# henry123-boy/Level-S2FM_official

Measured on AMD Instinct MI355X. Metric: rendered rays/sec (fwd+bwd), higher is better.
Workload: dtype f32; 1 GPU; C2: ETH3D bounds, 1024 rays x 128 samples per GPU, dual field, L16/F2/T19 hash grid, fwd+loss+bwd; rays_per_gpu=1024, samples_per_ray=128, dual_field=True, parallelism=dp1 (rays sharded by view)

## Files before the change

### include/ls2fm.h

```cpp
#ifndef LS2FM_H
#define LS2FM_H

#include <stdint.h>

#ifdef __cplusplus
extern "C" {
#endif

#define LS2FM_ABI_VERSION 13
#define LS2FM_MAX_LEVELS 16
#define LS2FM_HIDDEN 64
#define LS2FM_FEAT 16
#define LS2FM_VIEW_ENC 27

typedef enum ls2fm_status {
    LS2FM_OK = 0,
    LS2FM_ERR_INVALID_ARGUMENT = -1,
    LS2FM_ERR_UNSUPPORTED = -2,
    LS2FM_ERR_LAUNCH = -3,
    LS2FM_ERR_WORKSPACE = -4,
    LS2FM_ERR_STARVED = -5
} ls2fm_status;

typedef struct ls2fm_grid_desc {
// ... 547 lines not shown
                        const int64_t* row, int64_t n_rows, float* points, float* normals, float* colours, int64_t* pixel,
                        void* stream);

#define LS2FM_TEXTURE_TILE 16
#define LS2FM_TEXTURE_MAX_CLASSES 8
int ls2fm_texture_texels(const float* verts, int64_t n_verts, const int32_t* faces, int64_t n_faces, const int32_t* order,
                         const int32_t* rot, int32_t n_classes, const int32_t* class_log2_pitch, const int64_t* class_count,
                         int32_t gutter, int32_t size, int32_t row_begin, int32_t row_end, int32_t* face, float* point,
                         float* normal, float* uv, void* stream);
int ls2fm_texture_render(const int32_t* face_id, const float* bary, int32_t n_views, int32_t height, int32_t width, const float* uv,
                         int64_t n_faces, const float* texture, int32_t size, int32_t channels, const float* background, float* out,
                         void* stream);

int ls2fm_set_scatter_mode(int mode);
int ls2fm_get_scatter_mode(void);

int ls2fm_profile_enable(int on);
int ls2fm_profile_reset(void);
int ls2fm_profile_count(void);
const char* ls2fm_profile_name(int index);
int ls2fm_profile_get(int index, double* total_ms, int64_t* launches);

#ifdef __cplusplus
}
#endif
#endif
```

### level-s2fm_official_amd/csrc/bin_items.h

```cpp
#pragma once

#include "render_common.h"

namespace {

constexpr int kAccSlots = 2 << kSlabShift;
constexpr int kSlabBins = 128 << (13 - kSlabShift);
constexpr int kBins = kSlabBins;
#ifndef LS2FM_FILL_TILE
#define LS2FM_FILL_TILE 256
#endif
constexpr int kCountThreads = LS2FM_FILL_TILE;
constexpr int kFillThreads = LS2FM_FILL_TILE;
constexpr int kFillCap = kFillThreads * 17 / 4;
#ifndef LS2FM_FILL_WIN
#define LS2FM_FILL_WIN (LS2FM_FILL_TILE * 17 / 8)
#endif
constexpr int kFillWin = LS2FM_FILL_WIN;
#ifndef LS2FM_ACC_THREADS
#define LS2FM_ACC_THREADS 1024
#endif
constexpr int kAccThreads = LS2FM_ACC_THREADS;
#ifndef LS2FM_ACC_BATCH
#define LS2FM_ACC_BATCH 4
#endif
constexpr int kAccBatch = LS2FM_ACC_BATCH;
constexpr int kMaxParts = 16;

typedef unsigned long long u64;

struct __attribute__((aligned(16))) Item {
    uint32_t ij;
    float wx;
    float a0, a1, b0, b1;
    float c0, c1;
};

struct __attribute__((aligned(4))) ItemS {
    uint32_t ij;
    float v00, v01;
    float v10, v11;
};
// ... 278 lines not shown
```

### level-s2fm_official_amd/csrc/bin_scatter.hip

```cpp
#include <atomic>
#include <cstdlib>

#include "bin_items.h"
#include "side_jobs.h"

namespace {

#ifndef LS2FM_FILL_MINW
#define LS2FM_FILL_MINW 5
#endif
template <bool DUAL>
__global__ void __launch_bounds__(kFillThreads, LS2FM_FILL_MINW)
scatter_fill_kernel(LevelSet lv, FieldC fc, const float* __restrict__ center, const float* __restrict__ ray, int64_t n_points,
                    int64_t p_pad, int sshift, const float* __restrict__ rpt, const float* __restrict__ rec1,
                    const float* __restrict__ rec2, const float* __restrict__ ray_bound, int64_t n_rays, int64_t r_pad,
                    BinMeta bm, int level_base, int n_explicit, SideJobs sj) {
    typedef typename ItemOf<DUAL>::type ItemT;
    __shared__ int hist[kBins];
    __shared__ int lds_off[kBins];
    __shared__ int base[kBins];
    __shared__ int run_len[kBins];
    constexpr int kWin = DUAL ? kFillWin : kFillCap;
    constexpr int kItemBytes = kWin * (int)sizeof(ItemT);
    constexpr int kStageBytes = kItemBytes + 4 * kWin + (DUAL ? 4 * kWin : 0);
    constexpr int kRawBytes = kStageBytes > 4 * kTailArenaFloats ? kStageBytes : 4 * kTailArenaFloats;
    static_assert(kItemBytes % 16 == 0, "the index array behind the items is aligned");
    __shared__ __attribute__((aligned(16))) unsigned char s_raw[kRawBytes];
    ItemT* const s_items = reinterpret_cast<ItemT*>(s_raw);
    uint32_t* const s_gidx = reinterpret_cast<uint32_t*>(s_raw + kItemBytes);
// ... 9 lines not shown
    const int tid = threadIdx.x, lane = tid & 63, l = level_base + n_lv - 1 - y_lv;
    const int n_tiles_x = (int)gridDim.x;
    const int tile_x = (n_tiles_x & 7) == 0 ? ((int)blockIdx.x & 7) * (n_tiles_x >> 3) + ((int)blockIdx.x >> 3) : (int)blockIdx.x;
    if (tile_x == 0 && y_lv == 0) {
        if (tid == 0) *acc_claim(bm) = 0;
        for (int q = tid; q < LS2FM_MAX_LEVELS * kBins; q += kFillThreads) bm.part_ticket[q] = 0;
    }
    static_assert(kBins <= kFillThreads, "one thread per slab for the run offsets");
    int pre_base = 0;
    if (tid < kBins) {
        const int before = bm.tile[((int64_t)l * bm.n_tiles + tile_x) * kBins + tid];
        pre_base = bm.start[l * kBins + tid] + before;
    }
    for (int b = tid; b < kBins; b += kFillThreads) hist[b] = 0;
    __syncthreads();
    const LevelC L = make_level_c(lv, l, sshift);
    const int64_t i = (int64_t)tile_x * kFillThreads + tid;
    const bool live = i < n_points;
    uint32_t g[3] = {0u, 0u, 0u};
    float w[3] = {0.f, 0.f, 0.f}, d0 = 0.f, d1 = 0.f, r0 = 0.f, r1 = 0.f, e0 = 0.f, e1 = 0.f, qd[3] = {0.f, 0.f, 0.f};
    if (live) {
        const float4 a = reinterpret_cast<const float4*>(rpt)[2 * i];
        const float4 c = reinterpret_cast<const float4*>(rpt)[2 * i + 1];
        const float4 b = reinterpret_cast<const float4*>(rec1)[(int64_t)l * p_pad + i];
        const float x[3] = {a.x, a.y, a.z};
#pragma unroll
        for (int q = 0; q < 3; ++q) pos_fract(x[q], L.scale, g[q], w[q]);
        d0 = b.x; d1 = b.y; r0 = b.z; r1 = b.w;
        qd[0] = L.scale * a.w; qd[1] = L.scale * c.x; qd[2] = L.scale * c.y;
        if (DUAL) {
            const float2 e = reinterpret_cast<const float2*>(rec2)[(int64_t)l * p_pad + i];
// ... 194 lines not shown
            for (int o = 32; o > 0; o >>= 1) b = fmaxf(b, __shfl_xor(b, o, 64));
            if (lane == 0) red[tid >> 6] = b;
            __syncthreads();
            if (tid == 0) {
                float m = 0.f;
                for (int q = 0; q < kFillThreads / 64; ++q) m = fmaxf(m, red[q]);
                bm.level_bound[16 * which + l] = m;
            }
            __syncthreads();
        }
    }
}

struct SlabPlan {
    int first[LS2FM_MAX_LEVELS + 1];
    int parts[LS2FM_MAX_LEVELS];
    int scratch[LS2FM_MAX_LEVELS];
    int headroom_bits;
    int n_explicit;
};

constexpr int kMinHeadroomBits = 18;
__device__ __forceinline__ void add_fixed(u64* slot, float v, float to_fixed) {
    const double d = fma((double)v, (double)to_fixed, 6755399441055744.0);
    atomicAdd(slot, (u64)__double_as_longlong(d) - 0x4338000000000000ull);
}

__device__ __forceinline__ void quantum_of(float bound, int headroom_bits, float& to_fixed, double& to_float) {
    int e_bound = 0;
    if (bound > 0.f) (void)frexpf(bound, &e_bound);
    int shift = 62 - headroom_bits - e_bound;
    shift = shift > 126 ? 126 : (shift < -126 ? -126 : shift);
    to_fixed = ldexpf(1.0f, shift);
    to_float = ldexp(1.0, -shift);
}

#ifdef LS2FM_STAMPS
__device__ long long g_acc_stamps[8 * 4096];
#endif


template <bool DUAL, bool ADD_INTO>
__device__ __forceinline__ void combine_entry(const LevelSet& lv, const SlabPlan& plan, const BinMeta& bm, int sshift, float* __restrict__ dtable1,
                                              float* __restrict__ dtable2, int l, uint32_t slab, int entry, float bound1, float bound2) {
    constexpr int F = DUAL ? 4 : 2;
    const uint32_t lo = slab << sshift;
    const uint32_t hi = lo + (1u << sshift) < lv.size[l] ? lo + (1u << sshift) : lv.size[l];
    if (lo + (uint32_t)entry >= hi) return;
    const int parts = plan.parts[l];
    float to_fixed, to_fixed2;
    double to_float1, to_float2;
    quantum_of(bound1, plan.headroom_bits, to_fixed, to_float1);
    quantum_of(bound2, plan.headroom_bits, to_fixed2, to_float2);
    const int E = 1 << sshift;
    const u64* __restrict__ src = bm.part_acc + (size_t)(plan.scratch[l] + (int)slab * parts) * kAccSlots + entry;
    u64 tot[F];
#pragma unroll
    for (int f = 0; f < F; ++f) tot[f] = 0ull;
    constexpr int kCombineBatch = 4;
    for (int q0 = 0; q0 < parts; q0 += kCombineBatch) {
        u64 v[kCombineBatch][F];
#pragma unroll
// ... 220 lines not shown
            }
#pragma unroll
            for (int u = 0; u < kAccBatch; ++u)
                if (b0 + tid + u * kAccThreads < cur.j_hi) add_item(now[u], DUAL ? nowx[u] : 0.f);
            b0 += BT;
        } while (b0 < cur.j_hi);
        PACC_STAMP(cur.uid, 1);
        if (tid < 64) {
            asm volatile("s_waitcnt vmcnt(0)" : "+v"(claimed) :: "memory");
            if (tid == 0) s_claim = claimed;
        }
        lds_barrier();
        PACC_STAMP(cur.uid, 2);
        AccUnitRaw nraw = acc_unit_fetch<DUAL, true>(plan, bm, block_base, dyn_base + __builtin_amdgcn_readfirstlane(s_claim), dyn_end);
        const uint32_t size = lv.size[l];
        const uint32_t lo = cur.slab << sshift;
        const uint32_t hi = lo + (1u << sshift) < size ? lo + (1u << sshift) : size;
        if (cur.parts > 1 && combine) {
            if (!(ADD_INTO && cur.n_items == 0)) {
                uint4* mine = reinterpret_cast<uint4*>(bm.part_acc + (size_t)(plan.scratch[l] + cur.wg) * kAccSlots);
                const uint4 z = make_uint4(0u, 0u, 0u, 0u);
                for (int e = tid; e < kAccSlots / 2; e += kAccThreads) {
                    mine[e] = reinterpret_cast<const uint4*>(acc)[e];
                    reinterpret_cast<uint4*>(acc)[e] = z;
                }
                __syncthreads();
                if (tid == 0) {
                    __builtin_amdgcn_fence(__ATOMIC_RELEASE, "agent");
                    asm volatile("s_waitcnt vmcnt(0)" ::: "memory");
                    const int arrived = __hip_atomic_fetch_add(&bm.part_ticket[l * kBins + (int)cur.slab], 1, __ATOMIC_RELAXED, __HIP_MEMORY_SCOPE_AGENT);
                    const int last = arrived == cur.parts - 1;
                    if (last) __builtin_amdgcn_fence(__ATOMIC_ACQUIRE, "agent");
                    s_claim2 = last;
                }
                __syncthreads();
                if (s_claim2) {
                    for (int entry = tid; entry < E; entry += kAccThreads)
                        combine_entry<DUAL, ADD_INTO>(lv, plan, bm, sshift, dtable1, dtable2, l, cur.slab, entry, cur.bound1, cur.bound2);
                }
            }
        } else if (!(ADD_INTO && cur.n_items == 0)) {
            float* dst1 = dtable1 + 2ull * (lv.offset[l] + lo);
            float* dst2 = DUAL ? dtable2 + 2ull * (lv.offset[l] + lo) : nullptr;
            for (int entry = tid; entry < (int)(hi - lo); entry += kAccThreads) {
                u64 tot[F];
#pragma unroll
                for (int f = 0; f < F; ++f) { tot[f] = acc[f * E + entry]; acc[f * E + entry] = 0ull; }
                float2 v1 = make_float2((float)((double)(long long)tot[0] * to_float1), (float)((double)(long long)tot[1] * to_float1));
                float* d1 = dst1 + 2 * entry;
                if (cur.parts > 1) {
                    if (tot[0] != 0ull) atomicAdd(d1, v1.x);
                    if (tot[1] != 0ull) atomicAdd(d1 + 1, v1.y);
// ... 55 lines not shown
        while (n < grid->n_levels && n < kMaxExplicitLevels && (long long)grid->resolution[n] <= n_samples) ++n;
    if (n > kMaxExplicitLevels) n = kMaxExplicitLevels;
    if (n > grid->n_levels) n = grid->n_levels;
    return n;
}

size_t ls2fm_bin_counts_bytes() { return 0; }

bool ls2fm_bins_levels_fit(const ls2fm_grid_desc* grid, int dual) { return levels_fit(grid, ls2fm_slab_shift(dual)); }

int ls2fm_launch_scatter_fill(const ls2fm_grid_desc* grid, const FieldC& fc, const float* center, const float* ray, float* bins_ws,
                              int64_t n_points, int64_t p_pad, const float* rec1, const float* rec2, const float* rpt,
                              const float* ray_bound, int64_t n_rays, int dual, hipStream_t stream, int level_lo, int level_hi,
                              int n_explicit, const void* side_jobs) {
    const int64_t r_pad = (n_rays + 63) / 64 * 64;
    const int sshift = ls2fm_slab_shift(dual);
    const BinMeta bm = make_bin_meta(bins_ws, n_points);
    const LevelSet lv = make_level_set(grid);
    if (level_hi < 0) level_hi = grid->n_levels;
    if (level_hi <= level_lo) return LS2FM_OK;
    SideJobs sj{};
    if (side_jobs) {
        sj = *static_cast<const SideJobs*>(side_jobs);
        const int n_jobs = sj.dec_blocks + sj.l1_jobs + sj.n_red + kFinalizeTasks;
        sj.rows = (n_jobs + bm.n_tiles - 1) / bm.n_tiles;
    }
    if (kFillThreads != kWmThreads && sj.rows > 0) return LS2FM_ERR_UNSUPPORTED;
    const dim3 g((unsigned)bm.n_tiles, (unsigned)(level_hi - level_lo + sj.rows));
    if (dual) scatter_fill_kernel<true><<<g, kFillThreads, 0, stream>>>(lv, fc, center, ray, n_points, p_pad, sshift, rpt, rec1, rec2, ray_bound, n_rays, r_pad, bm, level_lo, n_explicit, sj);
    else      scatter_fill_kernel<false><<<g, kFillThreads, 0, stream>>>(lv, fc, center, ray, n_points, p_pad, sshift, rpt, rec1, nullptr, ray_bound, n_rays, r_pad, bm, level_lo, 0, sj);
    return ls2fm_launch_status();
}

namespace {
struct HostPlan { SlabPlan plan; int total, zero_lo, zero_hi; };

std::atomic<int> g_scatter_mode{[] { const char* e = getenv("LS2FM_SCATTER_MODE"); return e ? atoi(e) : 1; }()};

HostPlan make_plan(const ls2fm_grid_desc* grid, int64_t n_points, int sshift, int n_explicit = 0, int n_samples = 1) {
    const int capacity = part_blocks_capacity(n_points);
    for (int max_parts = kMaxParts;; --max_parts) {
        HostPlan h{};
        for (int l = 0; l < LS2FM_MAX_LEVELS; ++l) h.plan.parts[l] = 1;
        h.plan.headroom_bits = 4;
        while ((1ll << (h.plan.headroom_bits - 4)) < n_points) ++h.plan.headroom_bits;
        if (h.plan.headroom_bits < kMinHeadroomBits) h.plan.headroom_bits = kMinHeadroomBits;
        h.plan.n_explicit = n_explicit < LS2FM_MAX_LEVELS ? n_explicit : 0;
        h.zero_lo = h.zero_hi = -1;
        const int64_t target = 16384;
        int scratch = 0;
        for (int l = 0; l < LS2FM_MAX_LEVELS + 1; ++l) {
            h.plan.first[l] = h.total;
            if (l >= grid->n_levels) continue;
            const int slabs = level_slabs(grid->size[l], sshift);
            int parts = 1;
            if (!grid->hashed[l] || slabs < 16) {
                int64_t per_block = 4 * n_points / slabs;
                if (l < n_explicit) {
                    const double run = 0.9 * (double)n_samples / (double)grid->resolution[l];
                    if (run > 1.0) per_block = (int64_t)((double)per_block / run);
                }
                parts = (int)((per_block + target - 1) / target);
                if (parts > max_parts) parts = max_parts;
                if (parts < 1) parts = 1;
            }
            h.plan.parts[l] = parts;
            h.plan.scratch[l] = scratch;
            if (parts > 1) {
                scratch += slabs * parts;
                if (h.zero_lo < 0) h.zero_lo = l;
                h.zero_hi = l;
            }
            h.total += slabs * parts;
        }
        if (scratch <= capacity || max_parts == 1) return h;
    }
}
}

extern "C" int ls2fm_set_scatter_mode(int mode) {
    if (mode != 0 && mode != 1) return LS2FM_ERR_INVALID_ARGUMENT;
    g_scatter_mode.store(mode);
    return LS2FM_OK;
}
extern "C" int ls2fm_get_scatter_mode(void) { return g_scatter_mode.load(); }

void ls2fm_scatter_zero_range(const ls2fm_grid_desc* grid, int64_t n_points, bool dual, int64_t* first, int64_t* count) {
    const HostPlan h = make_plan(grid, n_points, ls2fm_slab_shift(dual ? 1 : 0));
    *first = 0; *count = 0;
    if (g_scatter_mode.load() != 0 || h.zero_lo < 0) return;
    *first = grid->offset[h.zero_lo];
    *count = (int64_t)grid->offset[h.zero_hi] + grid->size[h.zero_hi] - *first;
}

#ifdef LS2FM_STAMPS
extern "C" int ls2fm_debug_acc_stamps(long long* host) {
    return hipMemcpyFromSymbol(host, HIP_SYMBOL(g_acc_stamps), sizeof(long long) * 8 * 4096) == hipSuccess ? 0 : -1;
}
#endif

int ls2fm_launch_slab_accumulate(const ls2fm_grid_desc* grid, float* bins_ws, int64_t n_points, float* dtable1, float* dtable2,
                                 hipStream_t stream, int level_lo, int level_hi, int add_into, int n_explicit, int n_samples) {
    const bool dual = dtable2 != nullptr;
    const int sshift = ls2fm_slab_shift(dual ? 1 : 0);
    const BinMeta bm = make_bin_meta(bins_ws, n_points);
    const LevelSet lv = make_level_set(grid);
    const HostPlan h = make_plan(grid, n_points, sshift, dual ? n_explicit : LS2FM_MAX_LEVELS, n_samples);
    const int combine = g_scatter_mode.load() != 0 ? 1 : 0;
    if (level_hi < 0) level_hi = grid->n_levels;
    const int base = h.plan.first[level_lo], blocks = h.plan.first[level_hi] - base;
    if (blocks <= 0) return LS2FM_OK;
    static const int n_cus = [] {
        int dev = 0, n = 0;
        if (hipGetDevice(&dev) != hipSuccess || hipDeviceGetAttribute(&n, hipDeviceAttributeMultiprocessorCount, dev) != hipSuccess || n < 1) n = 256;
        return n;
    }();
    {
        const int g = blocks < n_cus ? blocks : n_cus;
        int* claim = acc_claim(bm);
        int hold = 0;
        for (int l = level_lo; l < level_hi && h.plan.parts[l] > 1; ++l) hold += h.plan.first[l + 1] - h.plan.first[l];
        if (hold > g || blocks < 3 * g) hold = 0;
// ... 12 lines not shown
```

### level-s2fm_official_amd/csrc/render_common.h

```cpp
#pragma once

#include "ls2fm_device.h"

enum ls2fm_prof_id {
    LS2FM_PROF_PREP = 0, LS2FM_PROF_ENCODE_SDF, LS2FM_PROF_ENCODE_RAD, LS2FM_PROF_SHADE_FWD, LS2FM_PROF_SHADE_BWD,
    LS2FM_PROF_WGRAD_GEO, LS2FM_PROF_WGRAD_TAIL, LS2FM_PROF_SCATTER_SDF, LS2FM_PROF_SCATTER_RAD, LS2FM_PROF_FINALIZE,
    LS2FM_PROF_SDF_EVAL, LS2FM_PROF_SPHERE_TRACE, LS2FM_PROF_BIN, LS2FM_PROF_LOSS_FWD,
    LS2FM_PROF_LOSS_BWD, LS2FM_PROF_WGRAD_MLP, LS2FM_PROF_POSE, LS2FM_PROF_ENCODE_PAIR,
    LS2FM_PROF_BALM_LINEARIZE, LS2FM_PROF_BALM_POINTS, LS2FM_PROF_BALM_SCHUR, LS2FM_PROF_BALM_SOLVE, LS2FM_PROF_BALM_BACKSUB,
    LS2FM_PROF_BALM_COST, LS2FM_PROF_COUNT
};
bool ls2fm_prof_enabled();
void ls2fm_prof_begin(int id, hipStream_t stream);
void ls2fm_prof_end(int id, hipStream_t stream);

struct SideCtx { hipStream_t side; hipEvent_t fork, mid, join; };
bool ls2fm_side_stream(SideCtx* out, hipStream_t caller);
int ls2fm_join_on_error(bool forked, const SideCtx& sc, hipStream_t caller, int status);
int* ls2fm_async_error_word(hipStream_t stream);
int ls2fm_device_cus();

constexpr int kHidden = LS2FM_HIDDEN;
constexpr int kOut = LS2FM_FEAT + 1;
constexpr int kInMax = 3 + 2 * LS2FM_MAX_LEVELS;
// ... 166 lines not shown
int ls2fm_explicit_levels(const ls2fm_grid_desc* grid, int dual, int n_samples);

struct WsLayout {
    int64_t p, p_pad, r_pad;
    int l1, l2, dual;
    int64_t packed, e1, j1, e2, sdfv, nrm, rgbs, fe, fe2, rout, lpart;
    int64_t rec1, rec2, rpt, bins, v, p3, gf, dz, gf2, dzr, renc, dexyz, dlen, mpart, wg, dbeta, smax;
    int64_t total;
};

#ifndef LS2FM_SLAB_SHIFT
#define LS2FM_SLAB_SHIFT 13
#endif
constexpr int kSlabShift = LS2FM_SLAB_SHIFT;
static inline int ls2fm_slab_shift(int dual) { return dual ? kSlabShift - 1 : kSlabShift; }
constexpr int kWgradMlpBlocks = 256;
constexpr int kRegsSdf = 48 + 16 + 16 + 5;
constexpr int kRegsGeo = 48 + 16 + 4;
constexpr int kRegsDec = 20;
constexpr int kL1Seg = 16;
struct WgPartLayout {
    int64_t l1_sdf;
    int64_t l1_geo;
    int64_t dec;
    int64_t slot_sdf;
    int64_t slot_geo;
    int64_t total;
    int n_slots;
};
static inline bool ls2fm_fused_wgrad(int n_samples) {
// ... 137 lines not shown
```

### level-s2fm_official_amd/csrc/render_fwd.hip

```cpp
#include <cmath>

#include "bin_items.h"

namespace {

struct LayerRef { const float* v; const float* g; const float* b; int out, in; };

__device__ __forceinline__ LayerRef layer_ref(const ls2fm_params& P, int li, int in_dim, int rad_in) {
    switch (li) {
        case 0: return {P.sdf_mlp[0].weight_v, P.sdf_mlp[0].weight_g, P.sdf_mlp[0].bias, kHidden, in_dim};
        case 1: return {P.sdf_mlp[1].weight_v, P.sdf_mlp[1].weight_g, P.sdf_mlp[1].bias, kOut, kHidden};
        case 2: return {P.geo_mlp[0].weight_v, P.geo_mlp[0].weight_g, P.geo_mlp[0].bias, kHidden, in_dim};
        case 3: return {P.geo_mlp[1].weight_v, P.geo_mlp[1].weight_g, P.geo_mlp[1].bias, kOut, kHidden};
        case 4: return {P.rad_mlp[0].weight_v, P.rad_mlp[0].weight_g, P.rad_mlp[0].bias, kHidden, rad_in};
        case 5: return {P.rad_mlp[1].weight_v, P.rad_mlp[1].weight_g, P.rad_mlp[1].bias, kHidden, kHidden};
        default: return {P.rad_mlp[2].weight_v, P.rad_mlp[2].weight_g, P.rad_mlp[2].bias, 3, kHidden};
    }
}

__device__ __forceinline__ int row_base(int li) {
    switch (li) {
        case 0: return 0;
        case 1: return 64;
        case 2: return 81;
// ... 195 lines not shown
    prep_weights_task(P, in_dim, in_dim2, rad_in, dual, with_rad, out, (int)blockIdx.x, (int)threadIdx.x, kPrepThreads);
}

struct XcdPlan { int start[9]; };

#ifdef LS2FM_STAMPS
__device__ unsigned long long g_enc_ticks[2 * LS2FM_MAX_LEVELS + 24];
#endif

struct EncodeExtras {
    ls2fm_params params;
    int in_dim, in_dim2, rad_in, dual;
    Packed* packed;
    int* tile_counts;
    int* scan_ticket;
    int n_tiles, sshift;
    int n_explicit;
    int n_prep_tasks;
    const float* pts;
};

constexpr int kEncThreads = 512;
constexpr int kEncRows = kEncThreads / kFillTile;
static_assert(kEncThreads % kFillTile == 0, "a gather workgroup covers whole tiles");
constexpr int kEncReserved = 8;

struct LevelOne { float scale; uint32_t res, size, offset, hashed; };

__device__ __forceinline__ void locate_sample(const FieldC& fc, const float* __restrict__ center, const float* __restrict__ ray,
                                              const float* __restrict__ pts, int64_t i, const LevelOne& lv, uint32_t g[3], Cell& c) {
    float p[3], x[3];
// ... 13 lines not shown
    for (int d = 0; d < 3; ++d) pos_fract(x[d], lv.scale, g[d], c.w[d]);
#pragma unroll
    for (int k = 0; k < 8; ++k)
        c.idx[k] = lv.offset + corner_index(g[0] + (k & 1), g[1] + ((k >> 1) & 1), g[2] + ((k >> 2) & 1), lv.res, lv.size,
                                            lv.hashed);
}

#ifndef LS2FM_ENC_MINW
#define LS2FM_ENC_MINW 1
#endif
template <bool INTERLEAVED>
__global__ void __launch_bounds__(kEncThreads, LS2FM_ENC_MINW)
ray_encode_kernel(LevelSet lv1, LevelSet lv2, FieldC fc, const float* __restrict__ center, const float* __restrict__ ray,
                  const float* __restrict__ table1, const float* __restrict__ table2, int64_t n_points, int64_t p_pad,
                  int n_chunks, XcdPlan plan, float* __restrict__ enc1, float* __restrict__ enc2, float* __restrict__ jac,
                  EncodeExtras ex) {
    __shared__ int hist[kEncRows][kBins];
    const int tid = threadIdx.x;
    if (blockIdx.x < kEncReserved) {
        if (ex.packed && (int)blockIdx.x < ex.n_prep_tasks)
            prep_weights_task(ex.params, ex.in_dim, ex.in_dim2, ex.rad_in, ex.dual, 1, ex.packed, (int)blockIdx.x, tid, kEncThreads);
        if (blockIdx.x == 3 && tid == 0 && ex.scan_ticket) *ex.scan_ticket = 0;
        return;
    }
    const int bx = (int)blockIdx.x - kEncReserved;
    const int xcd = bx & 7, j = bx >> 3;
    const int unit = plan.start[xcd] + j;
    if (unit >= plan.start[xcd + 1]) return;
    const int pl = unit / n_chunks;
    const int chunk = unit % n_chunks;
    const bool two = !INTERLEAVED && table2 != nullptr;
    const bool second = two && (pl & 1);
    const int l = two ? pl >> 1 : pl;
    LevelOne lv;
    lv.scale = second ? lv2.scale[l] : lv1.scale[l];
    lv.res = second ? lv2.res[l] : lv1.res[l];
    lv.size = second ? lv2.size[l] : lv1.size[l];
    lv.offset = second ? lv2.offset[l] : lv1.offset[l];
    lv.hashed = second ? lv2.hashed[l] : lv1.hashed[l];
    const bool counting = ex.tile_counts != nullptr && !second;
    if (counting) {
        for (int b = tid; b < kEncRows * kBins; b += kEncThreads) (&hist[0][0])[b] = 0;
        __syncthreads();
    }
    const int64_t i = (int64_t)chunk * kEncThreads + tid;
#ifdef LS2FM_STAMPS
    const long long t_begin = wall_clock64();
#endif
    if (i < n_points) {
        uint32_t g[3];
        Cell c;
        locate_sample(fc, center, ray, ex.pts, i, lv, g, c);
        auto enc_at = [=](float* __restrict__ base, int row, uint32_t k) -> float* { return base + ((int64_t)row * p_pad + i) * k; };
        if (INTERLEAVED) {
// ... 55 lines not shown
                    __builtin_nontemporal_store(lv.scale * g0, enc_at(jac, 2 * l + 0, 3u) + gd);
                    __builtin_nontemporal_store(lv.scale * g1, enc_at(jac, 2 * l + 1, 3u) + gd);
                }
            }
        }
        if (counting) {
            const bool factored = ex.dual != 0 && l >= ex.n_explicit;
            const int ray_len = ls2fm_ray_len_of_runs(ex.pts == nullptr, fc.n_samples);
            const uint32_t n_in_ray = ray_len != 0 ? (uint32_t)i % (uint32_t)ray_len : 0u;
            const RunFlags rf = wave_runs(g, true, tid & 63, factored ? kMergeMinDual : kMergeMinSingle, ray_len, n_in_ray);
            if (rf.head) {
                const bool halves = factored && rf.merged;
#pragma unroll
                for (int cp = 0; cp < 4; ++cp) {
                    const uint32_t i0 = c.idx[2 * cp] - lv.offset, i1 = c.idx[2 * cp + 1] - lv.offset;
                    const uint32_t s0 = i0 >> ex.sshift, s1 = i1 >> ex.sshift;
                    atomicAdd(&hist[tid / kFillTile][s0], 1);
                    if (s1 != s0 || halves) atomicAdd(&hist[tid / kFillTile][s1], 1);
                }
            }
        }
    }
    if (counting) {
        __syncthreads();
        for (int b = tid; b < kEncRows * kBins; b += kEncThreads) {
            const int tile = kEncRows * chunk + b / kBins;
            if (tile < ex.n_tiles) ex.tile_counts[((int64_t)l * ex.n_tiles + tile) * kBins + b % kBins] = hist[b / kBins][b % kBins];
        }
    }
#ifdef LS2FM_STAMPS
    __syncthreads();
// ... 118 lines not shown
int ls2fm_launch_points_encode(const ls2fm_field_desc* field, const ls2fm_grid_desc* grid, const ls2fm_params* params,
                               const float* pts, const WsLayout& w, float* ws, hipStream_t s) {
    const FieldC fc = make_field_c(field);
    const int L = grid->n_levels;
    const int n_chunks = (int)((w.p + kEncThreads - 1) / kEncThreads);
    int most = 0;
    const XcdPlan plan = make_xcd_plan(grid, L, nullptr, 0, 1, n_chunks, true, &most);
    EncodeExtras ex;
    ex.params = *params;
    ex.in_dim = 3 + 2 * L; ex.in_dim2 = 0; ex.rad_in = 0; ex.dual = 0;
    ex.packed = (Packed*)(ws + w.packed);
    const BinMeta bm = make_bin_meta(ws + w.bins, w.p);
    ex.tile_counts = bm.tile;
    ex.scan_ticket = scan_ticket(bm);
    ex.n_tiles = bm.n_tiles;
    ex.sshift = ls2fm_slab_shift(0);
    ex.n_explicit = 0;
    ex.n_prep_tasks = 1;
    ex.pts = pts;
    ray_encode_kernel<false><<<(unsigned)(kEncReserved + 8 * most), kEncThreads, 0, s>>>(
        make_level_set(grid), make_level_set(grid), fc, nullptr, nullptr, params->sdf_table, nullptr, w.p, w.p_pad, n_chunks, plan,
        ws + w.e1, nullptr, ws + w.j1, ex);
    return ls2fm_launch_status();
}
int ls2fm_launch_image_encode(const ls2fm_field_desc* field, const ls2fm_grid_desc* sdf_grid, const ls2fm_grid_desc* rad_grid,
                              const ls2fm_params* params, const float* center, const float* ray, int64_t n_points, int64_t p_pad,
                              float* e1, float* e2, float* j1, Packed* packed, hipStream_t s) {
    const FieldC fc = make_field_c(field);
    const int dual = field->dual_field ? 1 : 0;
    const int L1 = sdf_grid->n_levels, L2 = dual ? rad_grid->n_levels : 0;
    const int n_chunks = (int)((n_points + kEncThreads - 1) / kEncThreads);
    const bool interleaved = dual && params->dual_table;
    const bool pair = dual && !interleaved;
    int most = 0;
    const XcdPlan plan = make_xcd_plan(sdf_grid, L1, pair ? rad_grid : nullptr, pair ? L2 : 0, field->n_samples, n_chunks, false, &most,
                                       interleaved);
    EncodeExtras ex;
    ex.params = *params;
    ex.in_dim = 3 + 2 * L1; ex.in_dim2 = 3 + 2 * L2; ex.rad_in = 3 + 3 + kView + LS2FM_FEAT * (dual ? 2 : 1); ex.dual = dual;
    ex.packed = packed;
    ex.tile_counts = nullptr; ex.scan_ticket = nullptr; ex.n_tiles = 0; ex.sshift = ls2fm_slab_shift(dual);
    ex.n_explicit = 0;
    ex.n_prep_tasks = 3; ex.pts = nullptr;
    const unsigned enc_blocks = (unsigned)(kEncReserved + 8 * most);
    const int enc_span = dual ? LS2FM_PROF_ENCODE_PAIR : LS2FM_PROF_ENCODE_SDF;
    ls2fm_prof_begin(enc_span, s);
    if (interleaved)
        ray_encode_kernel<true><<<enc_blocks, kEncThreads, 0, s>>>(
            make_level_set(sdf_grid), make_level_set(sdf_grid), fc, center, ray, params->dual_table, nullptr, n_points, p_pad, n_chunks,
            plan, e1, e2, j1, ex);
    else
        ray_encode_kernel<false><<<enc_blocks, kEncThreads, 0, s>>>(
            make_level_set(sdf_grid), make_level_set(pair ? rad_grid : sdf_grid), fc, center, ray, params->sdf_table,
            pair ? params->rad_table : nullptr, n_points, p_pad, n_chunks, plan, e1, pair ? e2 : nullptr, j1, ex);
    ls2fm_prof_end(enc_span, s);
    return ls2fm_launch_status();
}

int ls2fm_launch_post_shade(const ls2fm_loss_spec* loss, const float* ray_part, int64_t n_rays, int n_samples,
                            const ls2fm_grid_desc* scan_grid, int64_t n_points, float* bins_ws, hipStream_t stream);

extern "C" int ls2fm_render_fwd(const ls2fm_field_desc* field, const ls2fm_grid_desc* sdf_grid,
                                const ls2fm_grid_desc* rad_grid, const ls2fm_params* params, const float* center,
                                const float* ray, int64_t n_rays, float* rgb, float* sdfs_volume, float* normals,
                                float* depth_mlp, float* normal_mlp, void* workspace, const ls2fm_render_opts* opts,
                                void* stream) {
    LS2FM_CHECK_ARG(render_config_ok(field, sdf_grid, rad_grid) && params && n_rays >= 0);
    if (field->bg_sdf) return LS2FM_ERR_UNSUPPORTED;
    if (field->dual_field && !same_grid_geometry(sdf_grid, rad_grid)) return LS2FM_ERR_UNSUPPORTED;
// ... 12 lines not shown
    float* ws = (float*)workspace;
    Packed* pk = (Packed*)(ws + w.packed);
    const FieldC fc = make_field_c(field);

    const int n_chunks = (int)((w.p + kEncThreads - 1) / kEncThreads);
    const bool interleaved = dual && params->dual_table;
    const bool pair = dual && !interleaved;
    const int enc_span = dual ? LS2FM_PROF_ENCODE_PAIR : LS2FM_PROF_ENCODE_SDF;
    int most = 0;
    const XcdPlan plan = make_xcd_plan(sdf_grid, L1, pair ? rad_grid : nullptr, pair ? L2 : 0, field->n_samples, n_chunks, prepare_bwd, &most,
                                       interleaved);
    EncodeExtras ex;
    ex.params = *params;
    ex.in_dim = 3 + 2 * L1; ex.in_dim2 = 3 + 2 * L2; ex.rad_in = 3 + 3 + kView + LS2FM_FEAT * (dual ? 2 : 1); ex.dual = dual;
    ex.packed = pk;
    ex.tile_counts = nullptr; ex.scan_ticket = nullptr; ex.n_tiles = 0; ex.sshift = ls2fm_slab_shift(dual);
    ex.n_explicit = ls2fm_explicit_levels(sdf_grid, dual, field->n_samples);
    ex.n_prep_tasks = 3; ex.pts = nullptr;
    if (prepare_bwd) {
        const BinMeta bm = make_bin_meta(ws + w.bins, w.p);
        ex.tile_counts = bm.tile;
        ex.scan_ticket = scan_ticket(bm);
        ex.n_tiles = bm.n_tiles;
    }
    const unsigned enc_blocks = (unsigned)(kEncReserved + 8 * most);
    ls2fm_prof_begin(enc_span, s);
    if (interleaved)
        ray_encode_kernel<true><<<enc_blocks, kEncThreads, 0, s>>>(
            make_level_set(sdf_grid), make_level_set(sdf_grid), fc, center, ray, params->dual_table, nullptr, w.p, w.p_pad, n_chunks,
            plan, ws + w.e1, ws + w.e2, ws + w.j1, ex);
    else
        ray_encode_kernel<false><<<enc_blocks, kEncThreads, 0, s>>>(
            make_level_set(sdf_grid), make_level_set(pair ? rad_grid : sdf_grid), fc, center, ray, params->sdf_table,
            pair ? params->rad_table : nullptr, w.p, w.p_pad, n_chunks, plan, ws + w.e1, pair ? ws + w.e2 : nullptr, ws + w.j1, ex);
    ls2fm_prof_end(enc_span, s);

    ls2fm_prof_begin(LS2FM_PROF_SHADE_FWD, s);
    ls2fm_launch_shade_fwd(fc, dual, 2 * L1, 2 * L2, pk, center, ray, n_rays, w, ws, rgb, sdfs_volume, normals, depth_mlp,
                           normal_mlp, loss, s);
    ls2fm_prof_end(LS2FM_PROF_SHADE_FWD, s);
    if (loss && opts->loss_inputs_ready && hipStreamWaitEvent(s, (hipEvent_t)opts->loss_inputs_ready, 0) != hipSuccess)
        return LS2FM_ERR_LAUNCH;
    ls2fm_prof_begin(LS2FM_PROF_BIN, s);
    const int st = ls2fm_launch_post_shade(loss, ws + w.lpart, n_rays, field->n_samples, prepare_bwd ? sdf_grid : nullptr, w.p,
                                           ws + w.bins, s);
    ls2fm_prof_end(LS2FM_PROF_BIN, s);
    if (st != LS2FM_OK) return st;
    return ls2fm_launch_status();
}
// ... 1 lines not shown
```

### level-s2fm_official_amd/ls2fm/_lib.py

```python
from __future__ import annotations

import ctypes
import os
from ctypes import POINTER, Structure, c_char_p, c_double, c_float, c_int32, c_int64, c_uint32, c_void_p

import torch

MAX_LEVELS = 16
HIDDEN = 64
FEAT = 16
ABI_VERSION = 13
MAX_RENDER_POINTS = 1 << 23

_HERE = os.path.dirname(os.path.abspath(__file__))
LIB_PATH = os.environ.get("LS2FM_LIB") or os.path.join(_HERE, "libls2fm_hip.so")


class GridDesc(Structure):
    _fields_ = [
        ("n_levels", c_int32),
        ("n_features", c_int32),
        ("scale", c_float * MAX_LEVELS),
        ("resolution", c_uint32 * MAX_LEVELS),
        ("size", c_uint32 * MAX_LEVELS),
# ... 239 lines not shown
                                   _P]),
    "ls2fm_mvs_plane_score": (c_int32, [_P, c_int32, c_int32, c_int32, _P, c_int32, _P, c_int32, _P, _P, c_int32, c_int32, c_float, c_float,
                                        c_int32, _P, _P, _P, _P]),
    "ls2fm_mvs_patchmatch_step": (c_int32, [_P, c_int32, c_int32, c_int32, _P, c_int32, _P, c_int32, _P, _P, c_int32, c_int32, c_float,
                                            c_float, c_int32, c_int32, c_int32, ctypes.c_uint32, c_float, c_float, c_float, _P, _P, _P, _P,
                                            _P, _P]),
    "ls2fm_mvs_fuse_mark": (c_int32, [_P, _P, c_int32, c_int32, c_int32, _P, c_int32, _P, _P, _P, c_float, c_float, c_float, c_float,
                                      c_int32, c_int32, _P, _P]),
    "ls2fm_mvs_fuse_emit": (c_int32, [_P, _P, _P, c_int32, c_int32, c_int32, c_int32, _P, c_int32, _P, _P, _P, _P, c_float, c_float,
                                      c_float, c_float, c_int32, c_int32, _P, _P, c_int64, _P, _P, _P, _P, _P]),
    "ls2fm_texture_texels": (c_int32, [_P, c_int64, _P, c_int64, _P, _P, c_int32, POINTER(c_int32), POINTER(c_int64), c_int32, c_int32,
                                       c_int32, c_int32, _P, _P, _P, _P, _P]),
    "ls2fm_texture_render": (c_int32, [_P, _P, c_int32, c_int32, c_int32, _P, c_int64, _P, c_int32, c_int32, POINTER(c_float), _P, _P]),
    "ls2fm_set_scatter_mode": (c_int32, [c_int32]),
    "ls2fm_get_scatter_mode": (c_int32, []),
    "ls2fm_profile_enable": (c_int32, [c_int32]),
    "ls2fm_profile_reset": (c_int32, []),
    "ls2fm_profile_count": (c_int32, []),
    "ls2fm_profile_name": (c_char_p, [c_int32]),
    "ls2fm_profile_get": (c_int32, [c_int32, POINTER(ctypes.c_double), POINTER(c_int64)]),
}
EXPORTED_SYMBOLS = tuple(_SIGNATURES)

_lib = None


def load() -> ctypes.CDLL:
    global _lib
    if _lib is not None:
        return _lib
# ... 82 lines not shown
```

Before: 2.559 million rays/s.

## Pick per-level slab shift to split heavily loaded dense levels into finer slabs

Replaces the single global slab shift with a per-level shift chosen by the host planner. For dense or small levels whose estimated items per slab exceed the unit target, the shift is lowered (down to a minimum, while the slab count fits in the bin array), which spreads hot dense-grid gradient accumulation across more slabs and fewer partial combines. The shifts are threaded through the fill, encode histogram and accumulate/combine kernels, and a diagnostic export of the plan is added. This costs extra host planning per launch and slightly larger kernel arguments, and if any kernel's slab indexing is not kept consistent it can bin items wrongly.

After: 2.576 million rays/s (median of 6 runs). About the same (+0.7%).

```diff
diff --git a/include/ls2fm.h b/include/ls2fm.h
--- a/include/ls2fm.h
+++ b/include/ls2fm.h
@@ -585,6 +585,7 @@
 
 int ls2fm_set_scatter_mode(int mode);
 int ls2fm_get_scatter_mode(void);
+int ls2fm_scatter_plan(const ls2fm_grid_desc* grid, int64_t n_points, int dual, int n_explicit, int n_samples, int32_t* out);
 
 int ls2fm_profile_enable(int on);
 int ls2fm_profile_reset(void);
diff --git a/level-s2fm_official_amd/csrc/bin_items.h b/level-s2fm_official_amd/csrc/bin_items.h
--- a/level-s2fm_official_amd/csrc/bin_items.h
+++ b/level-s2fm_official_amd/csrc/bin_items.h
@@ -26,6 +26,7 @@
 #endif
 constexpr int kAccBatch = LS2FM_ACC_BATCH;
 constexpr int kMaxParts = 16;
+constexpr int kMinSlabShift = 6;
 
 typedef unsigned long long u64;
 
diff --git a/level-s2fm_official_amd/csrc/bin_scatter.hip b/level-s2fm_official_amd/csrc/bin_scatter.hip
--- a/level-s2fm_official_amd/csrc/bin_scatter.hip
+++ b/level-s2fm_official_amd/csrc/bin_scatter.hip
@@ -12,7 +12,7 @@
 template <bool DUAL>
 __global__ void __launch_bounds__(kFillThreads, LS2FM_FILL_MINW)
 scatter_fill_kernel(LevelSet lv, FieldC fc, const float* __restrict__ center, const float* __restrict__ ray, int64_t n_points,
-                    int64_t p_pad, int sshift, const float* __restrict__ rpt, const float* __restrict__ rec1,
+                    int64_t p_pad, SlabShifts shifts, const float* __restrict__ rpt, const float* __restrict__ rec1,
                     const float* __restrict__ rec2, const float* __restrict__ ray_bound, int64_t n_rays, int64_t r_pad,
                     BinMeta bm, int level_base, int n_explicit, SideJobs sj) {
     typedef typename ItemOf<DUAL>::type ItemT;
@@ -52,7 +52,7 @@
     }
     for (int b = tid; b < kBins; b += kFillThreads) hist[b] = 0;
     __syncthreads();
-    const LevelC L = make_level_c(lv, l, sshift);
+    const LevelC L = make_level_c(lv, l, shifts.s[l]);
     const int64_t i = (int64_t)tile_x * kFillThreads + tid;
     const bool live = i < n_points;
     uint32_t g[3] = {0u, 0u, 0u};
@@ -277,6 +277,7 @@
 
 struct SlabPlan {
     int first[LS2FM_MAX_LEVELS + 1];
+    SlabShifts shift;
     int parts[LS2FM_MAX_LEVELS];
     int scratch[LS2FM_MAX_LEVELS];
     int headroom_bits;
@@ -307,8 +308,9 @@
 __device__ __forceinline__ void combine_entry(const LevelSet& lv, const SlabPlan& plan, const BinMeta& bm, int sshift, float* __restrict__ dtable1,
                                               float* __restrict__ dtable2, int l, uint32_t slab, int entry, float bound1, float bound2) {
     constexpr int F = DUAL ? 4 : 2;
-    const uint32_t lo = slab << sshift;
-    const uint32_t hi = lo + (1u << sshift) < lv.size[l] ? lo + (1u << sshift) : lv.size[l];
+    const int lshift = plan.shift.s[l];
+    const uint32_t lo = slab << lshift;
+    const uint32_t hi = lo + (1u << lshift) < lv.size[l] ? lo + (1u << lshift) : lv.size[l];
     if (lo + (uint32_t)entry >= hi) return;
     const int parts = plan.parts[l];
     float to_fixed, to_fixed2;
@@ -559,8 +561,9 @@
         PACC_STAMP(cur.uid, 2);
         AccUnitRaw nraw = acc_unit_fetch<DUAL, true>(plan, bm, block_base, dyn_base + __builtin_amdgcn_readfirstlane(s_claim), dyn_end);
         const uint32_t size = lv.size[l];
-        const uint32_t lo = cur.slab << sshift;
-        const uint32_t hi = lo + (1u << sshift) < size ? lo + (1u << sshift) : size;
+        const int lshift = plan.shift.s[l];
+        const uint32_t lo = cur.slab << lshift;
+        const uint32_t hi = lo + (1u << lshift) < size ? lo + (1u << lshift) : size;
         if (cur.parts > 1 && combine) {
             if (!(ADD_INTO && cur.n_items == 0)) {
                 uint4* mine = reinterpret_cast<uint4*>(bm.part_acc + (size_t)(plan.scratch[l] + cur.wg) * kAccSlots);
@@ -580,7 +583,7 @@
                 }
                 __syncthreads();
                 if (s_claim2) {
-                    for (int entry = tid; entry < E; entry += kAccThreads)
+                    for (int entry = tid; entry < (int)(hi - lo); entry += kAccThreads)
                         combine_entry<DUAL, ADD_INTO>(lv, plan, bm, sshift, dtable1, dtable2, l, cur.slab, entry, cur.bound1, cur.bound2);
                 }
             }
@@ -666,7 +669,7 @@
                               const float* ray_bound, int64_t n_rays, int dual, hipStream_t stream, int level_lo, int level_hi,
                               int n_explicit, const void* side_jobs) {
     const int64_t r_pad = (n_rays + 63) / 64 * 64;
-    const int sshift = ls2fm_slab_shift(dual);
+    const SlabShifts shifts = ls2fm_slab_shifts(grid, n_points, dual, n_explicit, fc.n_samples);
     const BinMeta bm = make_bin_meta(bins_ws, n_points);
     const LevelSet lv = make_level_set(grid);
     if (level_hi < 0) level_hi = grid->n_levels;
@@ -679,13 +682,14 @@
     }
     if (kFillThreads != kWmThreads && sj.rows > 0) return LS2FM_ERR_UNSUPPORTED;
     const dim3 g((unsigned)bm.n_tiles, (unsigned)(level_hi - level_lo + sj.rows));
-    if (dual) scatter_fill_kernel<true><<<g, kFillThreads, 0, stream>>>(lv, fc, center, ray, n_points, p_pad, sshift, rpt, rec1, rec2, ray_bound, n_rays, r_pad, bm, level_lo, n_explicit, sj);
-    else      scatter_fill_kernel<false><<<g, kFillThreads, 0, stream>>>(lv, fc, center, ray, n_points, p_pad, sshift, rpt, rec1, nullptr, ray_bound, n_rays, r_pad, bm, level_lo, 0, sj);
+    if (dual) scatter_fill_kernel<true><<<g, kFillThreads, 0, stream>>>(lv, fc, center, ray, n_points, p_pad, shifts, rpt, rec1, rec2, ray_bound, n_rays, r_pad, bm, level_lo, n_explicit, sj);
+    else      scatter_fill_kernel<false><<<g, kFillThreads, 0, stream>>>(lv, fc, center, ray, n_points, p_pad, shifts, rpt, rec1, nullptr, ray_bound, n_rays, r_pad, bm, level_lo, 0, sj);
     return ls2fm_launch_status();
 }
 
 namespace {
 struct HostPlan { SlabPlan plan; int total, zero_lo, zero_hi; };
+constexpr int kUnitItemTarget = 16384;
 
 std::atomic<int> g_scatter_mode{[] { const char* e = getenv("LS2FM_SCATTER_MODE"); return e ? atoi(e) : 1; }()};
 
@@ -699,23 +703,29 @@
         if (h.plan.headroom_bits < kMinHeadroomBits) h.plan.headroom_bits = kMinHeadroomBits;
         h.plan.n_explicit = n_explicit < LS2FM_MAX_LEVELS ? n_explicit : 0;
         h.zero_lo = h.zero_hi = -1;
-        const int64_t target = 16384;
+        const int64_t target = kUnitItemTarget;
         int scratch = 0;
         for (int l = 0; l < LS2FM_MAX_LEVELS + 1; ++l) {
             h.plan.first[l] = h.total;
             if (l >= grid->n_levels) continue;
-            const int slabs = level_slabs(grid->size[l], sshift);
+            int shift = sshift, slabs = level_slabs(grid->size[l], sshift);
             int parts = 1;
             if (!grid->hashed[l] || slabs < 16) {
-                int64_t per_block = 4 * n_points / slabs;
-                if (l < n_explicit) {
-                    const double run = 0.9 * (double)n_samples / (double)grid->resolution[l];
-                    if (run > 1.0) per_block = (int64_t)((double)per_block / run);
-                }
-                parts = (int)((per_block + target - 1) / target);
+                auto per_slab = [&](int s) {
+                    int64_t per = 4 * n_points / level_slabs(grid->size[l], s);
+                    if (l < n_explicit) {
+                        const double run = 0.9 * (double)n_samples / (double)grid->resolution[l];
+                        if (run > 1.0) per = (int64_t)((double)per / run);
+                    }
+                    return per;
+                };
+                while (shift > kMinSlabShift && per_slab(shift) > target && level_slabs(grid->size[l], shift - 1) <= kBins) --shift;
+                slabs = level_slabs(grid->size[l], shift);
+                parts = (int)((per_slab(shift) + target - 1) / target);
                 if (parts > max_parts) parts = max_parts;
                 if (parts < 1) parts = 1;
             }
+            h.plan.shift.s[l] = shift;
             h.plan.parts[l] = parts;
             h.plan.scratch[l] = scratch;
             if (parts > 1) {
@@ -728,6 +738,29 @@
         if (scratch <= capacity || max_parts == 1) return h;
     }
 }
+HostPlan plan_of(const ls2fm_grid_desc* grid, int64_t n_points, int dual, int n_explicit, int n_samples) {
+    return make_plan(grid, n_points, ls2fm_slab_shift(dual ? 1 : 0), dual ? n_explicit : LS2FM_MAX_LEVELS, n_samples);
+}
+}
+
+SlabShifts ls2fm_slab_shifts(const ls2fm_grid_desc* grid, int64_t n_points, int dual, int n_explicit, int n_samples) {
+    return plan_of(grid, n_points, dual, n_explicit, n_samples).plan.shift;
+}
+
+extern "C" int ls2fm_scatter_plan(const ls2fm_grid_desc* grid, int64_t n_points, int dual, int n_explicit, int n_samples, int32_t* out) {
+    LS2FM_CHECK_ARG(grid_desc_ok(grid) && n_points >= 0 && n_samples >= 1 && out);
+    const HostPlan h = plan_of(grid, n_points, dual, n_explicit, n_samples);
+    for (int q = 0; q < 96; ++q) out[q] = 0;
+    int used = 0;
+    for (int l = 0; l < grid->n_levels; ++l) {
+        const int slabs = level_slabs(grid->size[l], h.plan.shift.s[l]);
+        out[5 * l + 0] = h.plan.shift.s[l]; out[5 * l + 1] = slabs; out[5 * l + 2] = h.plan.parts[l];
+        out[5 * l + 3] = h.plan.first[l]; out[5 * l + 4] = h.plan.scratch[l];
+        if (h.plan.parts[l] > 1) used += slabs * h.plan.parts[l];
+    }
+    out[80] = h.total; out[81] = used; out[82] = part_blocks_capacity(n_points); out[83] = kBins; out[84] = kMinSlabShift;
+    out[85] = ls2fm_slab_shift(dual ? 1 : 0); out[86] = kUnitItemTarget;
+    return LS2FM_OK;
 }
 
 extern "C" int ls2fm_set_scatter_mode(int mode) {
@@ -757,7 +790,7 @@
     const int sshift = ls2fm_slab_shift(dual ? 1 : 0);
     const BinMeta bm = make_bin_meta(bins_ws, n_points);
     const LevelSet lv = make_level_set(grid);
-    const HostPlan h = make_plan(grid, n_points, sshift, dual ? n_explicit : LS2FM_MAX_LEVELS, n_samples);
+    const HostPlan h = plan_of(grid, n_points, dual ? 1 : 0, n_explicit, n_samples);
     const int combine = g_scatter_mode.load() != 0 ? 1 : 0;
     if (level_hi < 0) level_hi = grid->n_levels;
     const int base = h.plan.first[level_lo], blocks = h.plan.first[level_hi] - base;
diff --git a/level-s2fm_official_amd/csrc/render_common.h b/level-s2fm_official_amd/csrc/render_common.h
--- a/level-s2fm_official_amd/csrc/render_common.h
+++ b/level-s2fm_official_amd/csrc/render_common.h
@@ -204,6 +204,8 @@
 #endif
 constexpr int kSlabShift = LS2FM_SLAB_SHIFT;
 static inline int ls2fm_slab_shift(int dual) { return dual ? kSlabShift - 1 : kSlabShift; }
+struct SlabShifts { int32_t s[LS2FM_MAX_LEVELS]; };
+SlabShifts ls2fm_slab_shifts(const ls2fm_grid_desc* grid, int64_t n_points, int dual, int n_explicit, int n_samples);
 constexpr int kWgradMlpBlocks = 256;
 constexpr int kRegsSdf = 48 + 16 + 16 + 5;
 constexpr int kRegsGeo = 48 + 16 + 4;
diff --git a/level-s2fm_official_amd/csrc/render_fwd.hip b/level-s2fm_official_amd/csrc/render_fwd.hip
--- a/level-s2fm_official_amd/csrc/render_fwd.hip
+++ b/level-s2fm_official_amd/csrc/render_fwd.hip
@@ -233,7 +233,7 @@
     Packed* packed;
     int* tile_counts;
     int* scan_ticket;
-    int n_tiles, sshift;
+    int n_tiles;
     int n_explicit;
     int n_prep_tasks;
     const float* pts;
@@ -277,7 +277,7 @@
 ray_encode_kernel(LevelSet lv1, LevelSet lv2, FieldC fc, const float* __restrict__ center, const float* __restrict__ ray,
                   const float* __restrict__ table1, const float* __restrict__ table2, int64_t n_points, int64_t p_pad,
                   int n_chunks, XcdPlan plan, float* __restrict__ enc1, float* __restrict__ enc2, float* __restrict__ jac,
-                  EncodeExtras ex) {
+                  EncodeExtras ex, SlabShifts shifts) {
     __shared__ int hist[kEncRows][kBins];
     const int tid = threadIdx.x;
     if (blockIdx.x < kEncReserved) {
@@ -301,6 +301,7 @@
     lv.size = second ? lv2.size[l] : lv1.size[l];
     lv.offset = second ? lv2.offset[l] : lv1.offset[l];
     lv.hashed = second ? lv2.hashed[l] : lv1.hashed[l];
+    const int sshift = shifts.s[l];
     const bool counting = ex.tile_counts != nullptr && !second;
     if (counting) {
         for (int b = tid; b < kEncRows * kBins; b += kEncThreads) (&hist[0][0])[b] = 0;
@@ -386,7 +387,7 @@
 #pragma unroll
                 for (int cp = 0; cp < 4; ++cp) {
                     const uint32_t i0 = c.idx[2 * cp] - lv.offset, i1 = c.idx[2 * cp + 1] - lv.offset;
-                    const uint32_t s0 = i0 >> ex.sshift, s1 = i1 >> ex.sshift;
+                    const uint32_t s0 = i0 >> sshift, s1 = i1 >> sshift;
                     atomicAdd(&hist[tid / kFillTile][s0], 1);
                     if (s1 != s0 || halves) atomicAdd(&hist[tid / kFillTile][s1], 1);
                 }
@@ -535,13 +536,12 @@
     ex.tile_counts = bm.tile;
     ex.scan_ticket = scan_ticket(bm);
     ex.n_tiles = bm.n_tiles;
-    ex.sshift = ls2fm_slab_shift(0);
     ex.n_explicit = 0;
     ex.n_prep_tasks = 1;
     ex.pts = pts;
     ray_encode_kernel<false><<<(unsigned)(kEncReserved + 8 * most), kEncThreads, 0, s>>>(
         make_level_set(grid), make_level_set(grid), fc, nullptr, nullptr, params->sdf_table, nullptr, w.p, w.p_pad, n_chunks, plan,
-        ws + w.e1, nullptr, ws + w.j1, ex);
+        ws + w.e1, nullptr, ws + w.j1, ex, ls2fm_slab_shifts(grid, w.p, 0, 0, 1));
     return ls2fm_launch_status();
 }
 int ls2fm_launch_image_encode(const ls2fm_field_desc* field, const ls2fm_grid_desc* sdf_grid, const ls2fm_grid_desc* rad_grid,
@@ -560,7 +560,7 @@
     ex.params = *params;
     ex.in_dim = 3 + 2 * L1; ex.in_dim2 = 3 + 2 * L2; ex.rad_in = 3 + 3 + kView + LS2FM_FEAT * (dual ? 2 : 1); ex.dual = dual;
     ex.packed = packed;
-    ex.tile_counts = nullptr; ex.scan_ticket = nullptr; ex.n_tiles = 0; ex.sshift = ls2fm_slab_shift(dual);
+    ex.tile_counts = nullptr; ex.scan_ticket = nullptr; ex.n_tiles = 0;
     ex.n_explicit = 0;
     ex.n_prep_tasks = 3; ex.pts = nullptr;
     const unsigned enc_blocks = (unsigned)(kEncReserved + 8 * most);
@@ -569,11 +569,11 @@
     if (interleaved)
         ray_encode_kernel<true><<<enc_blocks, kEncThreads, 0, s>>>(
             make_level_set(sdf_grid), make_level_set(sdf_grid), fc, center, ray, params->dual_table, nullptr, n_points, p_pad, n_chunks,
-            plan, e1, e2, j1, ex);
+            plan, e1, e2, j1, ex, SlabShifts{});
     else
         ray_encode_kernel<false><<<enc_blocks, kEncThreads, 0, s>>>(
             make_level_set(sdf_grid), make_level_set(pair ? rad_grid : sdf_grid), fc, center, ray, params->sdf_table,
-            pair ? params->rad_table : nullptr, n_points, p_pad, n_chunks, plan, e1, pair ? e2 : nullptr, j1, ex);
+            pair ? params->rad_table : nullptr, n_points, p_pad, n_chunks, plan, e1, pair ? e2 : nullptr, j1, ex, SlabShifts{});
     ls2fm_prof_end(enc_span, s);
     return ls2fm_launch_status();
 }
@@ -616,8 +616,9 @@
     ex.params = *params;
     ex.in_dim = 3 + 2 * L1; ex.in_dim2 = 3 + 2 * L2; ex.rad_in = 3 + 3 + kView + LS2FM_FEAT * (dual ? 2 : 1); ex.dual = dual;
     ex.packed = pk;
-    ex.tile_counts = nullptr; ex.scan_ticket = nullptr; ex.n_tiles = 0; ex.sshift = ls2fm_slab_shift(dual);
+    ex.tile_counts = nullptr; ex.scan_ticket = nullptr; ex.n_tiles = 0;
     ex.n_explicit = ls2fm_explicit_levels(sdf_grid, dual, field->n_samples);
+    const SlabShifts shifts = ls2fm_slab_shifts(sdf_grid, w.p, dual, ex.n_explicit, field->n_samples);
     ex.n_prep_tasks = 3; ex.pts = nullptr;
     if (prepare_bwd) {
         const BinMeta bm = make_bin_meta(ws + w.bins, w.p);
@@ -630,11 +631,11 @@
     if (interleaved)
         ray_encode_kernel<true><<<enc_blocks, kEncThreads, 0, s>>>(
             make_level_set(sdf_grid), make_level_set(sdf_grid), fc, center, ray, params->dual_table, nullptr, w.p, w.p_pad, n_chunks,
-            plan, ws + w.e1, ws + w.e2, ws + w.j1, ex);
+            plan, ws + w.e1, ws + w.e2, ws + w.j1, ex, shifts);
     else
         ray_encode_kernel<false><<<enc_blocks, kEncThreads, 0, s>>>(
             make_level_set(sdf_grid), make_level_set(pair ? rad_grid : sdf_grid), fc, center, ray, params->sdf_table,
-            pair ? params->rad_table : nullptr, w.p, w.p_pad, n_chunks, plan, ws + w.e1, pair ? ws + w.e2 : nullptr, ws + w.j1, ex);
+            pair ? params->rad_table : nullptr, w.p, w.p_pad, n_chunks, plan, ws + w.e1, pair ? ws + w.e2 : nullptr, ws + w.j1, ex, shifts);
     ls2fm_prof_end(enc_span, s);
 
     ls2fm_prof_begin(LS2FM_PROF_SHADE_FWD, s);
diff --git a/level-s2fm_official_amd/ls2fm/_lib.py b/level-s2fm_official_amd/ls2fm/_lib.py
--- a/level-s2fm_official_amd/ls2fm/_lib.py
+++ b/level-s2fm_official_amd/ls2fm/_lib.py
@@ -277,6 +277,7 @@
     "ls2fm_texture_render": (c_int32, [_P, _P, c_int32, c_int32, c_int32, _P, c_int64, _P, c_int32, c_int32, POINTER(c_float), _P, _P]),
     "ls2fm_set_scatter_mode": (c_int32, [c_int32]),
     "ls2fm_get_scatter_mode": (c_int32, []),
+    "ls2fm_scatter_plan": (c_int32, [POINTER(GridDesc), c_int64, c_int32, c_int32, c_int32, POINTER(c_int32)]),
     "ls2fm_profile_enable": (c_int32, [c_int32]),
     "ls2fm_profile_reset": (c_int32, []),
     "ls2fm_profile_count": (c_int32, []),
```
